# 3dlg-hcvc/minsu3d

Hardware: AMD Instinct MI355X
Metric: scenes/sec (fwd+bwd) PointGroup on ~150k-pt 2cm voxels (higher is better)
Workload: dtype f32; 1 GPU; PointGroup m=16, synthetic ScanNet-shaped scenes (~144k points, ~106k voxels @2cm each), 4 scenes/GPU/step, grouping+ScoreNet branch on, fwd+loss+bwd+Adam; scenes_per_gpu=4, parallelism=dp1, grouping_inputs=GT labels, GT offsets + N(0,4cm) (random-init net groups nothing)

## Files before the change

minsu3d_amd/csrc/spconv.hip:

```cpp
#include <stdlib.h>
#include <atomic>
#include <map>
#include <mutex>
#include <unordered_map>
#include "common.h"
#include "../../include/minsu3d_hip.h"

typedef float f32x4 __attribute__((ext_vector_type(4)));

namespace {

constexpr int MAX_NBT = 8;
constexpr size_t LDS_BUDGET = 150 * 1024;
static hipError_t raise_lds_ceiling(const void *fn)
{
    hipFuncAttributes fa;
    hipError_t e = hipFuncGetAttributes(&fa, fn);
    if (e != hipSuccess) return e;
    return hipFuncSetAttribute(fn, hipFuncAttributeMaxDynamicSharedMemorySize, 160 * 1024 - (int)fa.sharedSizeBytes);
}

int env_int(const char *name, int dflt)
{
    const char *e = getenv(name);
    return e ? atoi(e) : dflt;
}

struct ConvArgs {
    const float *in;
    const float *wf;
    const float *wfs;
    const void *wfb;
    const int *nbr;
    float *out;
    const float *pre_scale;
    const float *pre_shift;
    const float *residual;
    const float *bias;
    const float *bn_x;
    const float *bn_scale;
    const float *bn_shift;
    const float *bn_mean;
    const float *bn_invstd;
    float *bn_partial;
    int out_stats;
    int Vout, K, Cin, Cout;
    int NCH;
    int NBtot;
    int G;
    int GC;
    int RT;
    int ntiles;
    int pre_relu;
    const int *pl_tile_start;
    const int *pl_entries;
    int dyn_picks;
    int k1_path;
    float *ws_slabs;
    unsigned *ws_cnt;
    int ws_ng, ws_kg, ws_R, ws_tpp;
};

__device__ __forceinline__ long stream_slot(long o, int NBtot)
{
    const int lane = (int)(o & 63);
    long r = o >> 6;
    const int nb = (int)(r % NBtot); r /= NBtot;
    const int t = (int)(r & 3); r >>= 2;
    return ((r * NBtot + nb) * 64 + lane) * 4 + t;
}

typedef __bf16 bf16x8 __attribute__((ext_vector_type(8)));

__host__ __device__ constexpr int aux_pieces(int aux_kind) { return aux_kind == 2 ? 3 : aux_kind == 3 ? 2 : aux_kind == 4 ? 1 : 0; }

__host__ __device__ inline bool bf3_dims_ok(int K, int Cin, int Cout)
{
    return K > 1 && Cin % 16 == 0 && Cout % 16 == 0 && Cin >= 48 && Cout >= 48 && Cin <= 256 && Cout <= 256;
}
// ... 417 lines not shown
{
    __syncthreads();
    float *dst = p.bn_partial + ((size_t)blockIdx.y * gridDim.x + blockIdx.x) * 2 * p.Cout;
    for (int t = threadIdx.x; t < 2 * p.Cout; t += blockDim.x) {
        const int which = t >= p.Cout, c = t - which * p.Cout - 16 * nb0;
        float sum = 0.f;
        if (c >= 0 && c < NBT * 16)
            for (int w = 0; w < nslots; w++) sum += s_part[(size_t)w * stat_slot_floats(NBT) + which * NBT * 16 + c];
        dst[t] = sum;
    }
}

template <int NBT>
__device__ __forceinline__ void store_tile(const ConvArgs &p, int row0, int nb0, f32x4 (&acc)[NBT], float *slot)
{
    const int l = lane_id(), q = l >> 4, jl = l & 15;
#pragma unroll
    for (int nb = 0; nb < NBT; nb++) {
        const int j = 16 * (nb0 + nb) + jl;
        const bool j_ok = j < p.Cout;
        float s1 = 0.f, s2 = 0.f;
#pragma unroll
        for (int r = 0; r < 4; r++) {
            const int row = row0 + 4 * q + r;
            if (row < p.Vout && j_ok) {
                float v = acc[nb][r];
                const size_t o = (size_t)row * p.Cout + j;
                if (p.residual) v += p.residual[o];
                if (p.bias) v += p.bias[j];
                if (p.bn_x) {
                    const float x = p.bn_x[o];
                    const float z = fmaf(x, p.bn_scale[j], p.bn_shift[j]);
                    v = (z > 0.f) ? v : 0.f;
                    s1 += v;
                    s2 += v * ((x - p.bn_mean[j]) * p.bn_invstd[j]);
                } else if (p.out_stats) {
                    s1 += v;
                    s2 = fmaf(v, v, s2);
                }
                p.out[o] = v;
            }
        }
        if (p.bn_x || p.out_stats) {
            s1 += __shfl_xor(s1, 16, 64); s1 += __shfl_xor(s1, 32, 64);
            s2 += __shfl_xor(s2, 16, 64); s2 += __shfl_xor(s2, 32, 64);
            if (q == 0) {
                slot[16 * nb + jl] += s1;
                slot[NBT * 16 + 16 * nb + jl] += s2;
            }
        }
    }
}

template <int NBT, bool ALIGNED, bool RES>
__global__ __launch_bounds__(1024) void spconv_fwd_kernel(ConvArgs p)
{
    extern __shared__ float lds[];
    const int l = lane_id(), q = l >> 4;
    const int waves = blockDim.x >> 6;
    const int nb0 = blockIdx.y * NBT;
    float *sW = lds;
    float *s_part = lds + (size_t)p.G * p.NCH * 4 * NBT * 64;
    const int slab4 = NBT * 16;
    auto stage = [&](int k_lo, int cnt) {
        const int rows = cnt * p.NCH * 4;
        for (int e = threadIdx.x; e < rows * slab4; e += blockDim.x) {
            const int r = e / slab4, c4 = e - r * slab4;
            reinterpret_cast<f32x4 *>(sW)[e] =
                reinterpret_cast<const f32x4 *>(p.wf + ((size_t)k_lo * p.NCH * 4 + r) * p.NBtot * 64 + (size_t)nb0 * 64)[c4];
        }
    };

    const bool with_partial = p.bn_x != nullptr || p.out_stats != 0;
    if (with_partial) stats_clear<NBT>(s_part, waves);
    float *slot = s_part + (size_t)wave_id() * stat_slot_floats(NBT);
    const int nblk = gridDim.x;
    const int per_xcd = (nblk + 7) / 8;
    int vb = (blockIdx.x % 8) * per_xcd + blockIdx.x / 8;
    if (nblk % 8 != 0) vb = blockIdx.x;

    if constexpr (RES) {
        stage(0, p.K);
        __syncthreads();
        const int total_waves = nblk * waves;
        const int chunk = (p.ntiles + total_waves - 1) / total_waves;
        const int wglobal = vb * waves + wave_id();
        const int t_begin = wglobal * chunk, t_end = min(p.ntiles, t_begin + chunk);
        for (int tile = t_begin; tile < t_end; tile++) {
            const int row0 = tile * 16;
            const int my_row = row0 + (l & 15);
            f32x4 acc[NBT];
#pragma unroll
            for (int nb = 0; nb < NBT; nb++) acc[nb] = (f32x4){0.f, 0.f, 0.f, 0.f};
            if (p.K == 1 && (p.k1_path & 1)) accumulate_k1<NBT, ALIGNED, false>(p, sW, my_row, q, nb0, acc);
            else accumulate_offsets<NBT, ALIGNED>(p, sW, 0, p.K, 0, my_row, q, nb0, acc);
            ConvArgs pt = p;
            asm volatile("" : "+s"(pt.out), "+s"(pt.residual), "+s"(pt.bias), "+s"(pt.bn_x), "+s"(pt.bn_scale), "+s"(pt.bn_shift),
                         "+s"(pt.bn_mean), "+s"(pt.bn_invstd));
            store_tile<NBT>(pt, row0, nb0, acc, slot);
        }
    } else {
        const int tile = vb * waves + wave_id();
        const int row0 = tile * 16;
        const int my_row = row0 + (l & 15);
        f32x4 acc[NBT];
#pragma unroll
        for (int nb = 0; nb < NBT; nb++) acc[nb] = (f32x4){0.f, 0.f, 0.f, 0.f};
        for (int g0 = 0; g0 < p.K; g0 += p.G) {
            const int gn = min(p.G, p.K - g0);
            __syncthreads();
            stage(g0, gn);
            __syncthreads();
            if (tile < p.ntiles) accumulate_offsets<NBT, ALIGNED>(p, sW, g0, g0 + gn, 0, my_row, q, nb0, acc);
        }
        if (tile < p.ntiles) store_tile<NBT>(p, row0, nb0, acc, slot);
    }
    if (with_partial) stats_flush<NBT>(p, s_part, waves, nb0);
}

constexpr int OGB = 5;

template <int NBT, int OG, int P = 3>
__global__ __launch_bounds__(1024) void spconv_fwd_bf3_kernel(ConvArgs p)
{
    extern __shared__ float lds[];
    const int l = lane_id(), g8 = l >> 4;
    const int waves = blockDim.x >> 6;
    const int nb0 = blockIdx.y * NBT;
    const int NC32 = (p.Cin + 31) >> 5;
    const int GC = p.GC > 0 ? p.GC : NC32;
    uint4 *sW = reinterpret_cast<uint4 *>(lds);
    const int slab = NBT * P * 64;
    float *s_part = lds + (size_t)p.G * GC * slab * 4;
    const uint4 *img = reinterpret_cast<const uint4 *>(p.wfb);
    auto stage = [&](int k_lo, int cnt, int c_lo, int ccnt) {
        uint4 *dst = sW;
        const int chunks = cnt * ccnt * NBT * P;
        for (int ch = wave_id(); ch < chunks; ch += waves) {
            const int r = ch / (NBT * P), within = ch - r * (NBT * P);
            const int kk = r / ccnt, cc = r - kk * ccnt;
            const uint4 *src = img + ((size_t)((k_lo + kk) * NC32 + c_lo + cc) * p.NBtot + nb0) * P * 64 + within * 64 + l;
            __builtin_amdgcn_global_load_lds((const __attribute__((address_space(1))) void *)src,
                                             (__attribute__((address_space(3))) void *)(dst + (size_t)ch * 64), 16, 0, 0);
        }
    };
    const bool with_partial = p.bn_x != nullptr || p.out_stats != 0;
    if (with_partial) stats_clear<NBT>(s_part, waves);
    const int nblk = gridDim.x;
    const int per_xcd = (nblk + 7) / 8;
    int vb = (blockIdx.x % 8) * per_xcd + blockIdx.x / 8;
    if (nblk % 8 != 0) vb = blockIdx.x;
    const bool affine = p.pre_scale != nullptr;
    const float relu_floor = p.pre_relu ? 0.f : -INFINITY;

    auto load_idx = [&](int k0, int k_end, int my_row, int (&idx)[OG]) {
        const bool row_ok = my_row < p.Vout;
        const int safe_row = row_ok ? my_row : 0;
#pragma unroll
        for (int u = 0; u < OG; u++) {
            const int k = min(k0 + u, p.K - 1);
            const int v = p.nbr[(size_t)k * p.Vout + safe_row];
            idx[u] = v | ((row_ok && k0 + u < k_end) ? 0 : -1);
        }
    };
    struct Round { f32x4 lo[OG], hi[OG]; };
    auto gather = [&](int c32, const int (&idx)[OG], Round &r) {
        const int cr = 32 * c32 + 8 * g8;
        const int c0 = cr < p.Cin ? cr : p.Cin - 8;
#pragma unroll
// ... 379 lines not shown
#pragma unroll
        for (int nb = 0; nb < NBT; nb++)
#pragma unroll
            for (int r = 0; r < 4; r++) s_acc[(((size_t)w * RT + t) * NBT + nb) * 256 + r * 64 + l] = acc[t][nb][r];
    __syncthreads();
    for (int t = w; t < RT; t += waves) {
        if (tile0 + t >= p.ntiles) break;
        f32x4 sum[NBT];
#pragma unroll
        for (int nb = 0; nb < NBT; nb++) sum[nb] = (f32x4){0.f, 0.f, 0.f, 0.f};
        for (int ww = 0; ww < waves; ww++)
#pragma unroll
            for (int nb = 0; nb < NBT; nb++)
#pragma unroll
                for (int r = 0; r < 4; r++) sum[nb][r] += s_acc[(((size_t)ww * RT + t) * NBT + nb) * 256 + r * 64 + l];
        store_tile<NBT>(p, (tile0 + t) * 16, nb0, sum, s_part + (size_t)w * stat_slot_floats(NBT));
    }
    if (with_partial) stats_flush<NBT>(p, s_part, waves, nb0);
}

template <int NBT, int RT, int P = 3>
int launch_fwd_small_bf3_rt(const ConvArgs &p, dim3 grid, int threads, size_t lds, hipStream_t stream)
{
    static const hipError_t attr = raise_lds_ceiling((const void *)spconv_fwd_small_bf3_rt_kernel<NBT, RT, P>);
    MS3D_CHECK(attr);
    spconv_fwd_small_bf3_rt_kernel<NBT, RT, P><<<grid, threads, lds, stream>>>(p);
    MS3D_LAUNCH_CHECK();
    return 0;
}

template <int NBT, int P = 3>
int launch_fwd_small_bf3(const ConvArgs &p, dim3 grid, int threads, size_t lds, hipStream_t stream)
{
    spconv_fwd_small_bf3_kernel<NBT, P><<<grid, threads, lds, stream>>>(p);
    MS3D_LAUNCH_CHECK();
    return 0;
}

template <int NBT>
int launch_fwd_small(const ConvArgs &p, dim3 grid, int threads, size_t lds, bool aligned, hipStream_t stream)
{
    if (aligned)
        spconv_fwd_small_kernel<NBT, true><<<grid, threads, lds, stream>>>(p);
    else
        spconv_fwd_small_kernel<NBT, false><<<grid, threads, lds, stream>>>(p);
    MS3D_LAUNCH_CHECK();
    return 0;
}

template <int NBT>
int launch_fwd(const ConvArgs &p, dim3 grid, int threads, size_t lds, bool aligned, hipStream_t stream)
{
    const bool res = p.G >= p.K;
#define MS3D_FWD_LAUNCH(A, R)                                                                                        \
    do {                                                                                                             \
        static const hipError_t attr = raise_lds_ceiling((const void *)spconv_fwd_kernel<NBT, A, R>);                \
        MS3D_CHECK(attr);                                                                                            \
        spconv_fwd_kernel<NBT, A, R><<<grid, threads, lds, stream>>>(p);                                             \
    } while (0)
    if (aligned && res) MS3D_FWD_LAUNCH(true, true);
    else if (aligned) MS3D_FWD_LAUNCH(true, false);
    else if (res) MS3D_FWD_LAUNCH(false, true);
    else MS3D_FWD_LAUNCH(false, false);
#undef MS3D_FWD_LAUNCH
    MS3D_LAUNCH_CHECK();
    return 0;
}


struct WsBlock { int u, g, nb0, k_lo, kcnt, t_begin, t_end; };

template <int NBT>
__device__ __forceinline__ bool ws_block(const ConvArgs &p, WsBlock &b)
{
    const int ny = p.NBtot / NBT, units = p.ws_R * ny;
    const int id = (int)blockIdx.x;
    b.u = (id / (8 * p.ws_ng)) * 8 + (id & 7);
    b.g = (id >> 3) % p.ws_ng;
    if (b.u >= units) return false;
    const int c = b.u % ny, r = b.u / ny;
    b.nb0 = c * NBT;
    b.k_lo = b.g * p.ws_kg;
    b.kcnt = min(p.K, b.k_lo + p.ws_kg) - b.k_lo;
    b.t_begin = r * p.ws_tpp;
    b.t_end = min(p.ntiles, b.t_begin + p.ws_tpp);
    return true;
}

__device__ __forceinline__ f32x4 *ws_slab_ptr(const ConvArgs &p, int g, int tile, int nb)
{
    return reinterpret_cast<f32x4 *>(p.ws_slabs) + (((size_t)g * p.ntiles + tile) * p.NBtot + nb) * 64 + lane_id();
}

template <int NBT>
__device__ __forceinline__ void ws_finish(const ConvArgs &p, const WsBlock &b, float *s_part, int *s_flag)
{
    const int w = wave_id(), waves = blockDim.x >> 6;
    const bool with_partial = p.bn_x != nullptr || p.out_stats != 0;
    if (p.ws_ng > 1) {
        asm volatile("s_waitcnt vmcnt(0)" ::: "memory");
        __syncthreads();
        if (threadIdx.x == 0) {
            __builtin_amdgcn_fence(__ATOMIC_RELEASE, "agent");
            asm volatile("s_waitcnt vmcnt(0)" ::: "memory");
            const unsigned t = __hip_atomic_fetch_add(&p.ws_cnt[b.u], 1u, __ATOMIC_RELAXED, __HIP_MEMORY_SCOPE_AGENT);
            const int last = t == (unsigned)(p.ws_ng - 1);
// ... 1396 lines not shown
#pragma unroll
            for (int b = 0; b < NA; b++)
#pragma unroll
                for (int r = 0; r < 4; r++) dst[b * 256 + r * 64 + l] = acc[b][r];
            if (l == 0) s_pk[w][n_partial] = k;
            n_partial++;
        }
    }
    if (pk0 >= 0) {
#pragma unroll
        for (int b = 0; b < NA; b++)
#pragma unroll
            for (int r = 0; r < 4; r++) s_tile[b * 256 + r * 64 + l] = part0[b][r];
        if (l == 0) s_pk[w][0] = pk0;
    }
    __syncthreads();
    for (int k = w; k < p.K; k += nw) {
        const bool empty = s_cum[k + 1] == s_cum[k];
        f32x4 acc[NA];
#pragma unroll
        for (int b = 0; b < NA; b++) acc[b] = (f32x4){0.f, 0.f, 0.f, 0.f};
        bool any = false;
        for (int ww = 0; ww < nw; ww++)
            for (int jj = 0; jj < 2; jj++)
                if (s_pk[ww][jj] == k) {
                    any = true;
                    const float *src = lds + (size_t)ww * WAVE_KB * 256 + (size_t)jj * NA * 256;
#pragma unroll
                    for (int b = 0; b < NA; b++)
#pragma unroll
                        for (int r = 0; r < 4; r++) acc[b][r] += src[b * 256 + r * 64 + l];
                }
        if (any || empty) store_slab(k, acc);
    }
}

template <int NBT, int NCH, int TB = WGRAD_TB>
int launch_wgrad_offsetlist(const WgradArgs &p, int nblk_rows, hipStream_t stream)
{
    constexpr int wave_kb = TB * (NCH + NBT) > 2 * NCH * NBT ? TB * (NCH + NBT) : 2 * NCH * NBT;
    const size_t per_wave = (size_t)wave_kb * 256 * sizeof(float);
    static const int max_w = env_int("MS3D_WGRAD_LIST_WAVES", 16);
    int nw = (int)(LDS_BUDGET / per_wave);
    if (nw > 16) nw = 16;
    if (nw > max_w && max_w >= 1) nw = max_w;
    dim3 grid(nblk_rows, ms3d_divup(p.NBtot, NBT), ms3d_divup(ms3d_divup(p.Cin, 16), NCH));
    const size_t lds = (size_t)nw * per_wave;
    static const hipError_t attr = raise_lds_ceiling((const void *)spconv_wgrad_offsetlist_kernel<NBT, NCH, TB>);
    MS3D_CHECK(attr);
    spconv_wgrad_offsetlist_kernel<NBT, NCH, TB><<<grid, nw * 64, lds, stream>>>(p);
    MS3D_LAUNCH_CHECK();
    return 0;
}

__global__ __launch_bounds__(1024) void bn_finalize_stats_kernel(const float *__restrict__ partial, int nparts, int C, long V,
                                                                float eps, float momentum, const float *__restrict__ gamma,
                                                                const float *__restrict__ beta, float *running_mean,
                                                                float *running_var, float *__restrict__ mean_out,
                                                                float *__restrict__ invstd_out, float *__restrict__ scale_out,
                                                                float *__restrict__ shift_out)
{
    __shared__ double s_1[16][17], s_2[16][17];
    const int cl = threadIdx.x & 15, lp = threadIdx.x >> 4;
    const int c = blockIdx.x * 16 + cl;
    double a1 = 0.0, a2 = 0.0;
    if (c < C) {
        int p = lp;
        for (; p + 192 < nparts; p += 256) {
            float v1[4], v2[4];
#pragma unroll
            for (int u = 0; u < 4; u++) {
                v1[u] = partial[((size_t)(p + 64 * u) * 2 + 0) * C + c];
                v2[u] = partial[((size_t)(p + 64 * u) * 2 + 1) * C + c];
            }
#pragma unroll
            for (int u = 0; u < 4; u++) {
                a1 += (double)v1[u];
                a2 += (double)v2[u];
            }
        }
        for (; p < nparts; p += 64) {
            a1 += (double)partial[((size_t)p * 2 + 0) * C + c];
            a2 += (double)partial[((size_t)p * 2 + 1) * C + c];
        }
    }
    a1 += __shfl_xor(a1, 16, 64); a2 += __shfl_xor(a2, 16, 64);
    a1 += __shfl_xor(a1, 32, 64); a2 += __shfl_xor(a2, 32, 64);
    if ((threadIdx.x & 63) < 16) {
        s_1[threadIdx.x >> 6][cl] = a1;
        s_2[threadIdx.x >> 6][cl] = a2;
    }
    __syncthreads();
    if (threadIdx.x >= 16 || c >= C) return;
    double s1 = 0.0, s2 = 0.0;
#pragma unroll
    for (int i = 0; i < 16; i++) {
        s1 += s_1[i][cl];
        s2 += s_2[i][cl];
    }
    const double mean = s1 / (double)V;
    double var = s2 / (double)V - mean * mean;
    if (var < 0.0) var = 0.0;
    const float invstd = (float)(1.0 / sqrt(var + (double)eps));
    const float g = gamma ? gamma[c] : 1.f, b = beta ? beta[c] : 0.f;
    mean_out[c] = (float)mean;
    invstd_out[c] = invstd;
// ... 777 lines not shown
int ms3d_spconv_pairlist_rows_dense(int Vout, int K, int Cin, int Cout)
{
    const int plain = ms3d_spconv_pairlist_rows(Vout, K, Cin, Cout);
    static const int narrow = env_int("MS3D_PL_NARROW", 1);
    if (plain != MS3D_PL_ROWS || !narrow || K != 27 || Cin != 32 || Cout != 32) return plain;
    const FwdGeom g = fwd_geometry(Vout, K, Cin, Cout, false, PL_ROWS_NARROW);
    return (g.ok && g.pairlist && g.pl_rows == PL_ROWS_NARROW) ? PL_ROWS_NARROW : plain;
}

int ms3d_spconv_partial_blocks(int Vout, int K, int Cin, int Cout, int with_pairlist)
{
    const FwdGeom g = fwd_geometry(Vout, K, Cin, Cout, true, with_pairlist == 1 ? MS3D_PL_ROWS : with_pairlist);
    return g.nblk * g.ny;
}

static int spconv_forward_impl(const float *in, const float *wf, const int *nbr, int Vout, int K, int Cin, int Cout,
                               float *out, const float *pre_scale, const float *pre_shift, int pre_relu,
                               const float *residual, const float *bn_x, const float *bn_scale, const float *bn_shift,
                               const float *bn_mean, const float *bn_invstd, float *bn_partial, int out_stats,
                               const float *bias, const int *pl_tile_start, const int *pl_entries, const float *wf_aux,
                               int aux_kind, ms3d_stream_t stream_);

int ms3d_spconv_forward(const float *in, const float *wf, const int *nbr, int Vout, int K, int Cin, int Cout,
                        float *out, const float *pre_scale, const float *pre_shift, int pre_relu,
                        const float *residual, const float *bn_x, const float *bn_scale, const float *bn_shift,
                        const float *bn_mean, const float *bn_invstd, float *bn_partial, int out_stats,
                        const float *bias, const int *pl_tile_start, const int *pl_entries, const float *wf_stream,
                        ms3d_stream_t stream_)
{
    return spconv_forward_impl(in, wf, nbr, Vout, K, Cin, Cout, out, pre_scale, pre_shift, pre_relu, residual, bn_x, bn_scale,
                               bn_shift, bn_mean, bn_invstd, bn_partial, out_stats, bias, pl_tile_start, pl_entries,
                               wf_stream, wf_stream ? 1 : 0, stream_);
}

static int spconv_forward_impl(const float *in, const float *wf, const int *nbr, int Vout, int K, int Cin, int Cout,
                               float *out, const float *pre_scale, const float *pre_shift, int pre_relu,
                               const float *residual, const float *bn_x, const float *bn_scale, const float *bn_shift,
                               const float *bn_mean, const float *bn_invstd, float *bn_partial, int out_stats,
                               const float *bias, const int *pl_tile_start, const int *pl_entries, const float *wf_stream,
                               int aux_kind, ms3d_stream_t stream_)
{
    hipStream_t stream = (hipStream_t)stream_;
    if (Vout <= 0) return 0;
    ConvArgs p;
    p.bias = bias;
    p.wfs = nullptr;
    p.wfb = nullptr;
    const int pieces = aux_pieces(aux_kind);
    if (aux_kind != 1 && !pieces) wf_stream = nullptr;
    p.pl_tile_start = pl_tile_start; p.pl_entries = pl_entries;
    p.out_stats = (out_stats && bn_partial && !bn_x) ? 1 : 0;
    static const int dyn_picks = [] { const char *e = getenv("MS3D_PL_DYNAMIC"); return e ? atoi(e) : 0; }();
    p.dyn_picks = dyn_picks;
    static const int k1_path = [] { const char *e = getenv("MS3D_K1_PATH"); return e ? atoi(e) : 3; }();
    p.k1_path = k1_path;
    p.in = in; p.wf = wf; p.nbr = nbr; p.out = out; p.pre_scale = pre_scale; p.pre_shift = pre_shift;
    p.residual = residual; p.bn_x = bn_x; p.bn_scale = bn_scale; p.bn_shift = bn_shift; p.bn_mean = bn_mean;
    p.bn_invstd = bn_invstd; p.bn_partial = bn_partial; p.Vout = Vout; p.K = K; p.Cin = Cin; p.Cout = Cout;
    p.NCH = ms3d_divup(Cin, 16); p.NBtot = ms3d_divup(Cout, 16); p.ntiles = ms3d_divup(Vout, 16); p.pre_relu = pre_relu;
    FwdPlan pl;
    const int rc = fwd_plan(Vout, K, Cin, Cout, (pl_tile_start && pl_entries) ? ms3d_kmap_pairlist_rows_of(pl_tile_start) : 0,
                            wf_stream ? aux_kind : 0, bn_x != nullptr || p.out_stats, pl);
    if (rc != 0) return rc;
    const FwdGeom &g = pl.g;
    p.G = pl.G;
    p.GC = pl.GC;
    p.RT = g.small ? g.rt : 1;
    dim3 grid(pl.grid_x, g.ny);
    const bool aligned = (Cin % 16 == 0);
    p.ws_slabs = nullptr; p.ws_cnt = nullptr; p.ws_ng = p.ws_kg = p.ws_R = p.ws_tpp = 0;
#define MS3D_BF_NBT(LAUNCH, P_, ...)                                                                                   \
    switch (g.nbt) {                                                                                                   \
        case 2: return LAUNCH<2, ##__VA_ARGS__, P_>(p, grid, g.threads, pl.lds, stream);                              \
        case 3: return LAUNCH<3, ##__VA_ARGS__, P_>(p, grid, g.threads, pl.lds, stream);                              \
        case 4: return LAUNCH<4, ##__VA_ARGS__, P_>(p, grid, g.threads, pl.lds, stream);                              \
        case 5: return LAUNCH<5, ##__VA_ARGS__, P_>(p, grid, g.threads, pl.lds, stream);                              \
        case 6: return LAUNCH<6, ##__VA_ARGS__, P_>(p, grid, g.threads, pl.lds, stream);                              \
        case 7: return LAUNCH<7, ##__VA_ARGS__, P_>(p, grid, g.threads, pl.lds, stream);                              \
        case 8: return LAUNCH<8, ##__VA_ARGS__, P_>(p, grid, g.threads, pl.lds, stream);                              \
    }
#define MS3D_BF_P(LAUNCH, ...)                                                                                         \
    if (pieces == 3) { MS3D_BF_NBT(LAUNCH, 3, ##__VA_ARGS__) }                                                         \
    else if (pieces == 2) { MS3D_BF_NBT(LAUNCH, 2, ##__VA_ARGS__) }                                                    \
    else { MS3D_BF_NBT(LAUNCH, 1, ##__VA_ARGS__) }
#define MS3D_F32_NBT(LAUNCH)                                                                                           \
    switch (g.nbt) {                                                                                                   \
        case 1: return LAUNCH<1>(p, grid, g.threads, pl.lds, aligned, stream);                                        \
        case 2: return LAUNCH<2>(p, grid, g.threads, pl.lds, aligned, stream);                                        \
        case 3: return LAUNCH<3>(p, grid, g.threads, pl.lds, aligned, stream);                                        \
        case 4: return LAUNCH<4>(p, grid, g.threads, pl.lds, aligned, stream);                                        \
        case 5: return LAUNCH<5>(p, grid, g.threads, pl.lds, aligned, stream);                                        \
        case 6: return LAUNCH<6>(p, grid, g.threads, pl.lds, aligned, stream);                                        \
        case 7: return LAUNCH<7>(p, grid, g.threads, pl.lds, aligned, stream);                                        \
        case 8: return LAUNCH<8>(p, grid, g.threads, pl.lds, aligned, stream);                                        \
    }
    switch (pl.family) {
        case FWD_WS: {
            WsSpace *sp = ws_space(stream, g.ws_ng > 1 ? (size_t)g.ws_ng * p.ntiles * p.NBtot * 256 : 0, g.ws_R * g.ny);
            if (!sp) return (int)hipErrorOutOfMemory;
            p.ws_slabs = sp->slabs; p.ws_cnt = sp->cnt;
            p.ws_ng = g.ws_ng; p.ws_kg = g.ws_kg; p.ws_R = g.ws_R; p.ws_tpp = g.ws_tpp;
            switch (g.nbt) {
                case 1: return launch_fwd_ws<1>(p, pl.grid_x, g.threads, pl.lds, stream);
                case 2: return launch_fwd_ws<2>(p, pl.grid_x, g.threads, pl.lds, stream);
                case 3: return launch_fwd_ws<3>(p, pl.grid_x, g.threads, pl.lds, stream);
                case 4: return launch_fwd_ws<4>(p, pl.grid_x, g.threads, pl.lds, stream);
            }
// ... 263 lines not shown
    int rc = wgrad_plan(Vout, K, Cin, Cout, ol_kt_start && ol_entries, submanifold, precision, plan);
    if (rc) return rc;
    const bool use_list = plan.route == WGRAD_LIST, wide2 = plan.wide2;
    p.ol_kt_start = ol_kt_start; p.ol_entries = ol_entries;
    p.rows_per_block = plan.rows_per_block;
    int nblk = plan.nblk;
    const int nb = p.NBtot;
    if (use_list) {
        const int nbs = nb <= 4 ? nb : ms3d_divup(nb, ms3d_divup(nb, 4));
        const bool two = ms3d_divup(Cin, 16) % 2 == 0 && nbs <= 2;
        rc = nbs == 1 ? (two ? launch_wgrad_offsetlist<1, 2>(p, nblk, stream) : launch_wgrad_offsetlist<1, 1>(p, nblk, stream))
           : nbs == 2 ? (two ? launch_wgrad_offsetlist<2, 2>(p, nblk, stream) : launch_wgrad_offsetlist<2, 1>(p, nblk, stream))
           : nbs == 3 ? launch_wgrad_offsetlist<3, 1>(p, nblk, stream)
                      : (wide2 ? launch_wgrad_offsetlist<4, 2, 1>(p, nblk, stream) : launch_wgrad_offsetlist<4, 1>(p, nblk, stream));
        if (rc) return rc;
        if (defer_nblk) { *defer_nblk = nblk; return 0; }
        launch_wgrad_reduce(partial_ws, nblk, n, dW, stream);
        MS3D_LAUNCH_CHECK();
        return 0;
    }
    if (plan.route == WGRAD_BF16) {
        const int P = 3 - precision;
        float *base = partial_ws + ms3d_spconv_wgrad_slab_floats(Vout, K, Cin, Cout);
        bf16x8 *img = reinterpret_cast<bf16x8 *>((reinterpret_cast<uintptr_t>(base) + 15) & ~(uintptr_t)15);
        const long ntile = ms3d_divup(Vout, 32);
        bf16x8 *xs = img + (size_t)ntile * nb * P * 64;
        const long t1 = ntile * nb * 64, t2 = (long)Vout * (Cin / 8);
        const int nb1 = (int)((t1 + 255) / 256), nb2 = (int)((t2 + 255) / 256);
        if (P == 3)
            wgrad_bf3_operands_kernel<3><<<nb1 + nb2, 256, 0, stream>>>(dout, in, Vout, Cin, Cout, nb, ntile, nb1, pre_scale,
                                                                       pre_shift, pre_relu, img, xs);
        else if (P == 2)
            wgrad_bf3_operands_kernel<2><<<nb1 + nb2, 256, 0, stream>>>(dout, in, Vout, Cin, Cout, nb, ntile, nb1, pre_scale,
                                                                       pre_shift, pre_relu, img, xs);
        else
            wgrad_bf3_operands_kernel<1><<<nb1 + nb2, 256, 0, stream>>>(dout, in, Vout, Cin, Cout, nb, ntile, nb1, pre_scale,
                                                                       pre_shift, pre_relu, img, xs);
        MS3D_LAUNCH_CHECK();
        WgradBf3Args q;
        q.xs = xs; q.dout_img = img; q.nbr = nbr; q.partial = partial_ws; q.Vout = Vout; q.K = K; q.Cin = Cin; q.Cout = Cout;
        q.NBtot = nb;
        q.rows_per_block = plan.rows_per_block;
#define MS3D_WG_BF(P_)                                                                                                 \
    (nb == 3 ? launch_wgrad_bf3<14, 3, 1, P_>(q, nblk, stream) : nb == 4 ? launch_wgrad_bf3<9, 4, 1, P_>(q, nblk, stream)   \
     : nb <= 6 ? launch_wgrad_bf3<9, 3, 2, P_>(q, nblk, stream) : launch_wgrad_bf3<9, 4, 2, P_>(q, nblk, stream))
        rc = P == 3 ? MS3D_WG_BF(3) : P == 2 ? MS3D_WG_BF(2) : MS3D_WG_BF(1);
#undef MS3D_WG_BF
        if (rc) return rc;
        if (defer_nblk) { *defer_nblk = nblk; return 0; }
        launch_wgrad_reduce(partial_ws, nblk, n, dW, stream);
        MS3D_LAUNCH_CHECK();
        return 0;
    }
    if (nb == 1) rc = (K >= 27) ? launch_wgrad<9, 1>(p, nblk, stream, dl) : launch_wgrad<8, 1>(p, nblk, stream, dl);
    else if (nb == 2) rc = (K >= 27) ? launch_wgrad<9, 2>(p, nblk, stream, dl) : launch_wgrad<8, 2>(p, nblk, stream, dl);
    else if (nb == 3) rc = (K >= 27) ? launch_wgrad<9, 3>(p, nblk, stream, dl) : launch_wgrad<8, 3>(p, nblk, stream, dl);
    else if (nb == 4) rc = launch_wgrad<4, 4>(p, nblk, stream, dl);
    else if (nb == 5) rc = launch_wgrad<4, 5>(p, nblk, stream, dl);
    else if (nb == 6) rc = launch_wgrad<4, 6>(p, nblk, stream, dl);
    else if (nb == 7) rc = launch_wgrad<4, 7>(p, nblk, stream, dl);
    else if (nb == 8) rc = launch_wgrad<3, 8>(p, nblk, stream, dl);
    else if (nb <= 10) rc = launch_wgrad<2, 10>(p, nblk, stream, dl);
    else if (nb <= 12) rc = launch_wgrad<2, 12>(p, nblk, stream, dl);
    else rc = launch_wgrad<2, 14>(p, nblk, stream, dl);
    if (rc) return rc;
    if (defer_nblk) { *defer_nblk = nblk; return 0; }
    launch_wgrad_reduce(partial_ws, nblk, n, dW, stream);
    MS3D_LAUNCH_CHECK();
    return 0;
}

size_t ms3d_spconv_wgrad_launch_bytes(void) { return 128; }

int ms3d_spconv_wgrad_multi(const void *descs, int n_desc, int total_blocks, int variant, ms3d_stream_t stream_)
{
    hipStream_t stream = (hipStream_t)stream_;
    if (n_desc <= 0 || total_blocks <= 0) return 0;
    switch (variant) {
#define MS3D_WM(KG, NBT) case KG * 100 + NBT: return launch_wgrad_multi<KG, NBT>(descs, n_desc, total_blocks, stream);
        MS3D_WM(9, 1) MS3D_WM(8, 1) MS3D_WM(9, 2) MS3D_WM(8, 2) MS3D_WM(9, 3) MS3D_WM(8, 3) MS3D_WM(4, 4) MS3D_WM(4, 5)
        MS3D_WM(4, 6) MS3D_WM(4, 7) MS3D_WM(3, 8) MS3D_WM(2, 10) MS3D_WM(2, 12) MS3D_WM(2, 14)
#undef MS3D_WM
    }
    return MS3D_E_UNSUPPORTED;
}

int ms3d_wgrad_reduce_blocks(long n, const float *slabs, const float *dW, int *wide)
{
    const bool w = n >= 32768 && (n & 3) == 0 && ((uintptr_t)slabs & 15) == 0 && ((uintptr_t)dW & 15) == 0;
    if (wide) *wide = w ? 1 : 0;
    return w ? ms3d_divup(n / 4, 64) : ms3d_divup(n, 16);
}

int ms3d_wgrad_reduce_multi(const void *descs, int n_desc, int total_blocks, ms3d_stream_t stream)
{
    if (n_desc <= 0 || total_blocks <= 0) return 0;
    wgrad_reduce_multi_kernel<<<total_blocks, 256, 0, (hipStream_t)stream>>>(static_cast<const WgradReduceDesc *>(descs),
                                                                           n_desc);
    MS3D_LAUNCH_CHECK();
    return 0;
}

int ms3d_bn_stats(const float *x, long V, int C, float eps, float momentum, const float *gamma, const float *beta,
                  float *running_mean, float *running_var, float *mean, float *invstd, float *scale, float *shift,
                  float *partial_ws, int partial_rows, ms3d_stream_t stream_)
{
    hipStream_t stream = (hipStream_t)stream_;
    if (V <= 0) return MS3D_E_UNSUPPORTED;
    int nblk = (int)((V + 255) / 256);
    if (nblk > partial_rows) nblk = partial_rows;
    if (nblk < 1) nblk = 1;
    const int rows_per_block = (int)((V + nblk - 1) / nblk);
    const int rc = launch_bn_partial_stats(x, V, C, partial_ws, nblk, rows_per_block, stream);
    if (rc) return rc;
    bn_finalize_stats_kernel<<<ms3d_divup(C, 16), 1024, 0, stream>>>(partial_ws, nblk, C, V, eps, momentum, gamma, beta,
                                                                  running_mean, running_var, mean, invstd, scale, shift);
    MS3D_LAUNCH_CHECK();
    return 0;
}

int ms3d_column_sum(const float *x, long V, int C, float *partial_ws, int partial_rows, float *out2c, ms3d_stream_t stream_)
{
    hipStream_t stream = (hipStream_t)stream_;
    if (V <= 0) {
        MS3D_CHECK(hipMemsetAsync(out2c, 0, sizeof(float) * 2 * C, stream));
        return 0;
    }
    int nblk = (int)((V + 1023) / 1024);
    if (nblk > partial_rows) nblk = partial_rows;
    if (nblk < 1) nblk = 1;
    const int rows_per_block = (int)((V + nblk - 1) / nblk);
    const int rc = launch_bn_partial_stats(x, V, C, partial_ws, nblk, rows_per_block, stream);
    if (rc) return rc;
    return ms3d_reduce_partials(partial_ws, nblk, 2 * C, out2c, stream_);
}
// ... 293 lines not shown
```

Baseline: 204.2 scenes/sec.

## Add dedicated software-pipelined kernels for 1x1 sparse conv forward and weight grad

Adds specialised kernels for K=1 (pointwise) sparse convolutions. In forward, each wave handles a contiguous chunk of tiles with weights staged in LDS once, and prefetches the next tile's neighbour index and input rows while the current tile runs MFMA. In weight-grad, a 4-wave kernel double-buffers gathered input and dout rows and reduces across waves in LDS. Both are turned on by default through a new k1_path default of 15. The cost is more code and template instances, and the forward uses a different grid mapping that could hurt occupancy.

```diff
diff --git a/minsu3d_amd/csrc/spconv.hip b/minsu3d_amd/csrc/spconv.hip
--- a/minsu3d_amd/csrc/spconv.hip
+++ b/minsu3d_amd/csrc/spconv.hip
@@ -25,6 +25,7 @@
     const char *e = getenv(name);
     return e ? atoi(e) : dflt;
 }
+constexpr int MS3D_K1_PATH_DEFAULT = 15;
 
 struct ConvArgs {
     const float *in;
@@ -548,6 +549,183 @@
     }
 }
 
+template <int NBT, bool ALIGNED>
+__device__ __forceinline__ void k1_tile_loop(const ConvArgs &p, const float *__restrict__ sW, int t_begin, int t_end, int nb0,
+                                             float *slot)
+{
+    constexpr int CB = 4;
+    const int l = lane_id(), q = l >> 4, i = l & 15;
+    if (t_begin >= t_end) return;
+    int opaque0 = 0;
+    asm volatile("" : "+s"(opaque0));
+    const bool wide = (p.Cout & 3) == 0 &&
+                      ((reinterpret_cast<uintptr_t>(p.out) | reinterpret_cast<uintptr_t>(p.residual) |
+                        reinterpret_cast<uintptr_t>(p.bn_x) | reinterpret_cast<uintptr_t>(p.bias) |
+                        reinterpret_cast<uintptr_t>(p.bn_scale) | reinterpret_cast<uintptr_t>(p.bn_shift) |
+                        reinterpret_cast<uintptr_t>(p.bn_mean) | reinterpret_cast<uintptr_t>(p.bn_invstd)) & 15) == 0;
+    auto entry = [&](int tile) -> int {
+        const int row = tile * 16 + i;
+        return p.nbr[min(row, p.Vout - 1)] | (row < p.Vout ? 0 : -1);
+    };
+    auto fetch = [&](int idx, int ch0, f32x4 (&a)[CB]) {
+        const float *row = p.in + (size_t)max(idx, 0) * p.Cin + 4 * q;
+#pragma unroll
+        for (int u = 0; u < CB; u++) {
+            const int ch = min(ch0 + u, p.NCH - 1);
+            if (ALIGNED) {
+                a[u] = *reinterpret_cast<const f32x4 *>(row + 16 * ch);
+            } else {
+#pragma unroll
+                for (int t = 0; t < 4; t++) a[u][t] = (16 * ch + 4 * q + t < p.Cin) ? row[16 * ch + t] : 0.f;
+            }
+        }
+    };
+    auto multiply = [&](int ch0, f32x4 (&a)[CB], int keep, f32x4 (&acc)[NBT]) {
+#pragma unroll
+        for (int u = 0; u < CB; u++) {
+            if (ch0 + u >= p.NCH) break;
+            const int ch = ch0 + u, c0 = 16 * ch + 4 * q;
+            if (p.pre_scale) {
+                f32x4 sc, sh;
+                if (ALIGNED) {
+                    sc = *reinterpret_cast<const f32x4 *>(p.pre_scale + c0);
+                    sh = *reinterpret_cast<const f32x4 *>(p.pre_shift + c0);
+                } else {
+#pragma unroll
+                    for (int t = 0; t < 4; t++) {
+                        sc[t] = (c0 + t < p.Cin) ? p.pre_scale[c0 + t] : 0.f;
+                        sh[t] = (c0 + t < p.Cin) ? p.pre_shift[c0 + t] : 0.f;
+                    }
+                }
+#pragma unroll
+                for (int t = 0; t < 4; t++) {
+                    const float v = fmaf(a[u][t], sc[t], sh[t]);
+                    a[u][t] = p.pre_relu ? fmaxf(v, 0.f) : v;
+                }
+            }
+#pragma unroll
+            for (int t = 0; t < 4; t++) a[u][t] = __int_as_float(__float_as_int(a[u][t]) & keep);
+            const float *w = sW + (size_t)(ch * 4) * NBT * 64 + l;
+#pragma unroll
+            for (int t = 0; t < 4; t++)
+#pragma unroll
+                for (int nb = 0; nb < NBT; nb++)
+                    acc[nb] = __builtin_amdgcn_mfma_f32_16x16x4f32(w[(t * NBT + nb) * 64], a[u][t], acc[nb], 0, 0, 0);
+        }
+    };
+    f32x4 st1[NBT], st2[NBT];
+#pragma unroll
+    for (int nb = 0; nb < NBT; nb++) st1[nb] = st2[nb] = (f32x4){0.f, 0.f, 0.f, 0.f};
+
+    int idx_n = entry(t_begin);
+    f32x4 a_n[CB];
+    fetch(idx_n, 0, a_n);
+    int idx_nn = entry(t_begin + 1 + opaque0);
+    for (int tile = t_begin; tile < t_end; tile++) {
+        const int idx = idx_n, keep = ~(idx >> 31);
+        f32x4 a[CB];
+#pragma unroll
+        for (int u = 0; u < CB; u++) a[u] = a_n[u];
+        idx_n = idx_nn;
+        fetch(idx_n, 0, a_n);
+        idx_nn = entry(tile + 2 + opaque0);
+        const int row = tile * 16 + i;
+        const bool row_ok = row < p.Vout;
+        const size_t orow = (size_t)min(row, p.Vout - 1) * p.Cout;
+        f32x4 acc[NBT];
+#pragma unroll
+        for (int nb = 0; nb < NBT; nb++) acc[nb] = (f32x4){0.f, 0.f, 0.f, 0.f};
+        if (__ballot(idx >= 0) != 0ull) {
+            multiply(0, a, keep, acc);
+            for (int ch0 = CB; ch0 < p.NCH; ch0 += CB) {
+                f32x4 b[CB];
+                fetch(idx, ch0, b);
+                multiply(ch0, b, keep, acc);
+            }
+        }
+        f32x4 res[NBT], bx[NBT];
+        if (wide) {
+#pragma unroll
+            for (int nb = 0; nb < NBT; nb++) {
+                const int j0 = 16 * (nb0 + nb) + 4 * q, js = j0 < p.Cout ? j0 : 0;
+                if (p.residual) res[nb] = *reinterpret_cast<const f32x4 *>(p.residual + orow + js);
+                if (p.bn_x) bx[nb] = *reinterpret_cast<const f32x4 *>(p.bn_x + orow + js);
+            }
+        }
+#pragma unroll
+        for (int nb = 0; nb < NBT; nb++) {
+            const int j0 = 16 * (nb0 + nb) + 4 * q;
+            if (wide) {
+                if (row_ok && j0 < p.Cout) {
+                    f32x4 v = acc[nb];
+                    if (p.residual) v += res[nb];
+                    if (p.bias) v += *reinterpret_cast<const f32x4 *>(p.bias + j0);
+                    if (p.bn_x) {
+                        const f32x4 sc = *reinterpret_cast<const f32x4 *>(p.bn_scale + j0);
+                        const f32x4 sh = *reinterpret_cast<const f32x4 *>(p.bn_shift + j0);
+                        const f32x4 mu = *reinterpret_cast<const f32x4 *>(p.bn_mean + j0);
+                        const f32x4 is = *reinterpret_cast<const f32x4 *>(p.bn_invstd + j0);
+#pragma unroll
+                        for (int r = 0; r < 4; r++) {
+                            const float x = bx[nb][r];
+                            const float z = fmaf(x, sc[r], sh[r]);
+                            v[r] = (z > 0.f) ? v[r] : 0.f;
+                            st1[nb][r] += v[r];
+                            st2[nb][r] += v[r] * ((x - mu[r]) * is[r]);
+                        }
+                    } else if (p.out_stats) {
+#pragma unroll
+                        for (int r = 0; r < 4; r++) {
+                            st1[nb][r] += v[r];
+                            st2[nb][r] = fmaf(v[r], v[r], st2[nb][r]);
+                        }
+                    }
+                    *reinterpret_cast<f32x4 *>(p.out + orow + j0) = v;
+                }
+            } else {
+#pragma unroll
+                for (int r = 0; r < 4; r++) {
+                    const int j = j0 + r;
+                    if (row_ok && j < p.Cout) {
+                        float v = acc[nb][r];
+                        const size_t o = orow + j;
+                        if (p.residual) v += p.residual[o];
+                        if (p.bias) v += p.bias[j];
+                        if (p.bn_x) {
+                            const float x = p.bn_x[o];
+                            const float z = fmaf(x, p.bn_scale[j], p.bn_shift[j]);
+                            v = (z > 0.f) ? v : 0.f;
+                            st1[nb][r] += v;
+                            st2[nb][r] += v * ((x - p.bn_mean[j]) * p.bn_invstd[j]);
+                        } else if (p.out_stats) {
+                            st1[nb][r] += v;
+                            st2[nb][r] = fmaf(v, v, st2[nb][r]);
+                        }
+                        p.out[o] = v;
+                    }
+                }
+            }
+        }
+    }
+    if (p.bn_x || p.out_stats) {
+#pragma unroll
+        for (int nb = 0; nb < NBT; nb++)
+#pragma unroll
+            for (int r = 0; r < 4; r++) {
+                float s1 = st1[nb][r], s2 = st2[nb][r];
+#pragma unroll
+                for (int m = 1; m < 16; m <<= 1) {
+                    s1 += __shfl_xor(s1, m, 64);
+                    s2 += __shfl_xor(s2, m, 64);
+                }
+                if (i == 0) {
+                    slot[16 * nb + 4 * q + r] += s1;
+                    slot[NBT * 16 + 16 * nb + 4 * q + r] += s2;
+                }
+            }
+    }
+}
+
 template <int NBT, bool ALIGNED, bool RES>
 __global__ __launch_bounds__(1024) void spconv_fwd_kernel(ConvArgs p)
 {
@@ -611,6 +789,37 @@
         }
         if (tile < p.ntiles) store_tile<NBT>(p, row0, nb0, acc, slot);
     }
+    if (with_partial) stats_flush<NBT>(p, s_part, waves, nb0);
+}
+
+constexpr int K1_LOOP_MAX_THREADS = 512;
+constexpr bool k1_loop_serves(int nbt) { return nbt == 1 || nbt == 2 || nbt == 4; }
+template <int NBT, bool ALIGNED>
+__global__ __launch_bounds__(K1_LOOP_MAX_THREADS, NBT <= 2 ? 4 : 2) void spconv_fwd_k1_kernel(ConvArgs p)
+{
+    extern __shared__ float lds[];
+    const int waves = blockDim.x >> 6;
+    const int nb0 = blockIdx.y * NBT;
+    float *sW = lds;
+    float *s_part = lds + (size_t)p.NCH * 4 * NBT * 64;
+    const int rows = p.NCH * 4, slab4 = NBT * 16;
+    for (int e = threadIdx.x; e < rows * slab4; e += blockDim.x) {
+        const int r = e / slab4, c4 = e - r * slab4;
+        reinterpret_cast<f32x4 *>(sW)[e] = reinterpret_cast<const f32x4 *>(p.wf + (size_t)r * p.NBtot * 64 + (size_t)nb0 * 64)[c4];
+    }
+    const bool with_partial = p.bn_x != nullptr || p.out_stats != 0;
+    if (with_partial) stats_clear<NBT>(s_part, waves);
+    float *slot = s_part + (size_t)wave_id() * stat_slot_floats(NBT);
+    const int nblk = gridDim.x;
+    const int per_xcd = (nblk + 7) / 8;
+    int vb = (blockIdx.x % 8) * per_xcd + blockIdx.x / 8;
+    if (nblk % 8 != 0) vb = blockIdx.x;
+    __syncthreads();
+    const int total_waves = nblk * waves;
+    const int chunk = (p.ntiles + total_waves - 1) / total_waves;
+    const int wglobal = vb * waves + wave_id();
+    const int t_begin = wglobal * chunk, t_end = min(p.ntiles, t_begin + chunk);
+    k1_tile_loop<NBT, ALIGNED>(p, sW, t_begin, t_end, nb0, slot);
     if (with_partial) stats_flush<NBT>(p, s_part, waves, nb0);
 }
 
@@ -1096,6 +1305,14 @@
 int launch_fwd(const ConvArgs &p, dim3 grid, int threads, size_t lds, bool aligned, hipStream_t stream)
 {
     const bool res = p.G >= p.K;
+    if constexpr (k1_loop_serves(NBT)) {
+        if (res && p.K == 1 && (p.k1_path & 5) == 5 && threads <= K1_LOOP_MAX_THREADS && lds <= 64 * 1024) {
+            if (aligned) spconv_fwd_k1_kernel<NBT, true><<<grid, threads, lds, stream>>>(p);
+            else spconv_fwd_k1_kernel<NBT, false><<<grid, threads, lds, stream>>>(p);
+            MS3D_LAUNCH_CHECK();
+            return 0;
+        }
+    }
 #define MS3D_FWD_LAUNCH(A, R)                                                                                        \
     do {                                                                                                             \
         static const hipError_t attr = raise_lds_ceiling((const void *)spconv_fwd_kernel<NBT, A, R>);                \
@@ -2598,6 +2815,223 @@
     MS3D_LAUNCH_CHECK();
     return 0;
 }
+
+constexpr int WGRAD_K1_WAVES = 4;
+constexpr int wgrad_k1_tb(int nbt, int nch) { return nch + nbt >= 6 ? 1 : 2; }
+constexpr int wgrad_k1_wave_kb(int nbt, int nch)
+{
+    return wgrad_k1_tb(nbt, nch) * (nch + nbt) > nch * nbt ? wgrad_k1_tb(nbt, nch) * (nch + nbt) : nch * nbt;
+}
+constexpr int wgrad_k1_variant(int nbt, int nch) { return 10000 + nch * 100 + nbt; }
+
+template <int NBT, int NCH>
+__device__ __forceinline__ void wgrad_k1_body(const WgradArgs &p, const int bx, const int bz, float *lds)
+{
+    constexpr int TB = wgrad_k1_tb(NBT, NCH), NT = NCH + NBT, NA = NCH * NBT, WAVE_KB = wgrad_k1_wave_kb(NBT, NCH);
+    constexpr int nw = WGRAD_K1_WAVES;
+    const int l = lane_id(), q = l >> 4, cl = l & 15, w = wave_id();
+    float *s_tile = lds + (size_t)w * WAVE_KB * 256;
+    const int qs = q ^ ((cl >> 1) & 3);
+    const int cbase = bz * NCH * 16;
+    const bool vec = ((p.Cin | p.Cout) & 3) == 0 &&
+                     ((reinterpret_cast<uintptr_t>(p.in) | reinterpret_cast<uintptr_t>(p.dout)) & 15) == 0;
+    f32x4 sc[NCH], sh[NCH];
+#pragma unroll
+    for (int ch = 0; ch < NCH; ch++)
+#pragma unroll
+        for (int i = 0; i < 4; i++) {
+            const int c = cbase + 16 * ch + 4 * q + i;
+            const bool ok = p.pre_scale && c < p.Cin;
+            sc[ch][i] = ok ? p.pre_scale[c] : 1.f;
+            sh[ch][i] = ok ? p.pre_shift[c] : 0.f;
+        }
+    const int r_begin = bx * p.rows_per_block;
+    const int r_end = min(p.Vout, r_begin + p.rows_per_block);
+    const int nbatch = (r_end - r_begin + 15) >> 4;
+    int opaque0 = 0;
+    asm volatile("" : "+s"(opaque0));
+    f32x4 acc[NA];
+#pragma unroll
+    for (int b = 0; b < NA; b++) acc[b] = (f32x4){0.f, 0.f, 0.f, 0.f};
+
+    int e[TB], erow[TB];
+    int gk[TB], grow[TB];
+    f32x4 ga[TB][NCH], gb[TB][NBT];
+    auto load_entries = [&](int bt) {
+#pragma unroll
+        for (int t = 0; t < TB; t++) {
+            erow[t] = min(r_begin + 16 * (bt + t) + cl, r_end - 1);
+            e[t] = p.nbr[erow[t]];
+        }
+    };
+    auto gather = [&]() {
+#pragma unroll
+        for (int t = 0; t < TB; t++) {
+            gk[t] = e[t];
+            grow[t] = erow[t];
+            const float *xi = p.in + (size_t)max(e[t], 0) * p.Cin;
+            const float *dy = p.dout + (size_t)erow[t] * p.Cout;
+            if (vec) {
+#pragma unroll
+                for (int ch = 0; ch < NCH; ch++) {
+                    const int c0 = cbase + 16 * ch + 4 * q;
+                    ga[t][ch] = *reinterpret_cast<const f32x4 *>(xi + (c0 < p.Cin ? c0 : 0));
+                }
+#pragma unroll
+                for (int nb = 0; nb < NBT; nb++) {
+                    const int j0 = 16 * nb + 4 * q;
+                    gb[t][nb] = *reinterpret_cast<const f32x4 *>(dy + (j0 < p.Cout ? j0 : 0));
+                }
+            } else {
+#pragma unroll
+                for (int ch = 0; ch < NCH; ch++)
+#pragma unroll
+                    for (int i = 0; i < 4; i++) ga[t][ch][i] = xi[min(cbase + 16 * ch + 4 * q + i, p.Cin - 1)];
+#pragma unroll
+                for (int nb = 0; nb < NBT; nb++)
+#pragma unroll
+                    for (int i = 0; i < 4; i++) gb[t][nb][i] = dy[min(16 * nb + 4 * q + i, p.Cout - 1)];
+            }
+        }
+    };
+    const int step = nw * TB, bt0 = w * TB;
+    if (bt0 < nbatch) {
+        load_entries(bt0);
+        gather();
+        load_entries(bt0 + step + opaque0);
+    }
+    for (int bt = bt0; bt < nbatch; bt += step) {
+        f32x4 ca[TB][NCH], cb[TB][NBT];
+        int ck[TB], crow[TB];
+#pragma unroll
+        for (int t = 0; t < TB; t++) {
+            ck[t] = gk[t];
+            crow[t] = grow[t];
+#pragma unroll
+            for (int ch = 0; ch < NCH; ch++) ca[t][ch] = ga[t][ch];
+#pragma unroll
+            for (int nb = 0; nb < NBT; nb++) cb[t][nb] = gb[t][nb];
+        }
+        gather();
+        load_entries(bt + 2 * step + opaque0);
+#pragma unroll
+        for (int t = 0; t < TB; t++) {
+            const bool row_ok = r_begin + 16 * (bt + t) + cl == crow[t];
+            const bool in_ok = row_ok && ck[t] >= 0;
+            float *ta = s_tile + (size_t)t * NT * 256;
+#pragma unroll
+            for (int ch = 0; ch < NCH; ch++) {
+#pragma unroll
+                for (int i = 0; i < 4; i++) {
+                    float v = ca[t][ch][i];
+                    if (p.pre_scale) {
+                        v = fmaf(v, sc[ch][i], sh[ch][i]);
+                        if (p.pre_relu) v = fmaxf(v, 0.f);
+                    }
+                    ca[t][ch][i] = (in_ok && cbase + 16 * ch + 4 * q + i < p.Cin) ? v : 0.f;
+                }
+                *reinterpret_cast<f32x4 *>(ta + ch * 256 + cl * 16 + 4 * qs) = ca[t][ch];
+            }
+#pragma unroll
+            for (int nb = 0; nb < NBT; nb++) {
+#pragma unroll
+                for (int i = 0; i < 4; i++) cb[t][nb][i] = (row_ok && 16 * nb + 4 * q + i < p.Cout) ? cb[t][nb][i] : 0.f;
+                *reinterpret_cast<f32x4 *>(ta + (NCH + nb) * 256 + cl * 16 + 4 * qs) = cb[t][nb];
+            }
+        }
+#pragma unroll
+        for (int t = 0; t < TB; t++) {
+            const float *ta = s_tile + (size_t)t * NT * 256;
+#pragma unroll
+            for (int st = 0; st < 4; st++) {
+                const int o = (4 * st + q) * 16 + (cl ^ (((2 * st + (q >> 1)) & 3) << 2));
+                float bv[NBT];
+#pragma unroll
+                for (int nb = 0; nb < NBT; nb++) bv[nb] = ta[(NCH + nb) * 256 + o];
+#pragma unroll
+                for (int ch = 0; ch < NCH; ch++) {
+                    const float av = ta[ch * 256 + o];
+#pragma unroll
+                    for (int nb = 0; nb < NBT; nb++)
+                        acc[ch * NBT + nb] = __builtin_amdgcn_mfma_f32_16x16x4f32(av, bv[nb], acc[ch * NBT + nb], 0, 0, 0);
+                }
+            }
+        }
+    }
+#pragma unroll
+    for (int b = 0; b < NA; b++)
+#pragma unroll
+        for (int r = 0; r < 4; r++) s_tile[b * 256 + r * 64 + l] = acc[b][r];
+    __syncthreads();
+    float *dst = p.partial + (size_t)bx * p.Cin * p.Cout;
+    for (int o = threadIdx.x; o < NA * 256; o += nw * 64) {
+        float v = 0.f;
+#pragma unroll
+        for (int ww = 0; ww < nw; ww++) v += lds[(size_t)ww * WAVE_KB * 256 + o];
+        const int b = o >> 8, r = (o >> 6) & 3, ln = o & 63;
+        const int ci = cbase + 16 * (b / NBT) + 4 * (ln >> 4) + r, j = 16 * (b % NBT) + (ln & 15);
+        if (ci < p.Cin && j < p.Cout) dst[(size_t)ci * p.Cout + j] = v;
+    }
+}
+
+template <int NBT, int NCH>
+__global__ __launch_bounds__(64 * WGRAD_K1_WAVES) void spconv_wgrad_k1_kernel(WgradArgs p, const unsigned char *__restrict__ descs,
+                                                                              int n_desc)
+{
+    extern __shared__ float lds[];
+    int bx = blockIdx.x, bz = blockIdx.z;
+    if (descs) {
+        int lo = 0, hi = n_desc - 1;
+        const int blk = blockIdx.x;
+        while (lo < hi) {
+            const int mid = (lo + hi + 1) >> 1;
+            if (reinterpret_cast<const WgradLaunch *>(descs + 128 * (size_t)mid)->block_begin <= blk) lo = mid; else hi = mid - 1;
+        }
+        const WgradLaunch *d = reinterpret_cast<const WgradLaunch *>(descs + 128 * (size_t)lo);
+        const int local = blk - d->block_begin;
+        bx = local % d->gx;
+        bz = local / (d->gx * d->gy);
+        p = d->p;
+    }
+    wgrad_k1_body<NBT, NCH>(p, bx, bz, lds);
+}
+
+template <int NBT, int NCH>
+int launch_wgrad_k1(const WgradArgs &p, int nblk_rows, hipStream_t stream, WgradLaunch *defer = nullptr)
+{
+    dim3 grid(nblk_rows, 1, ms3d_divup(ms3d_divup(p.Cin, 16), NCH));
+    if (defer) {
+        defer->block_begin = 0;
+        defer->gx = grid.x; defer->gy = grid.y; defer->gz = grid.z;
+        defer->variant = wgrad_k1_variant(NBT, NCH);
+        defer->nblk = nblk_rows;
+        defer->p = p;
+        return 0;
+    }
+    const size_t lds = (size_t)WGRAD_K1_WAVES * wgrad_k1_wave_kb(NBT, NCH) * 1024;
+    spconv_wgrad_k1_kernel<NBT, NCH><<<grid, 64 * WGRAD_K1_WAVES, lds, stream>>>(p, nullptr, 0);
+    MS3D_LAUNCH_CHECK();
+    return 0;
+}
+
+template <int NBT, int NCH>
+int launch_wgrad_k1_multi(const void *descs, int n_desc, int total_blocks, hipStream_t stream)
+{
+    const size_t lds = (size_t)WGRAD_K1_WAVES * wgrad_k1_wave_kb(NBT, NCH) * 1024;
+    WgradArgs none = {};
+    spconv_wgrad_k1_kernel<NBT, NCH><<<total_blocks, 64 * WGRAD_K1_WAVES, lds, stream>>>(none, static_cast<const unsigned char *>(descs),
+                                                                                       n_desc);
+    MS3D_LAUNCH_CHECK();
+    return 0;
+}
+
+static int wgrad_k1_nch(int Cin, int nb)
+{
+    if (nb > 8) return 0;
+    const int cap = nb <= 2 ? 4 : nb <= 4 ? 2 : 1, nch = ms3d_divup(Cin, 16);
+    return nch >= 4 ? cap : nch >= 2 ? (cap < 2 ? cap : 2) : 1;
+}
+#define MS3D_WK1_ALL(X) X(1, 1) X(1, 2) X(1, 4) X(2, 1) X(2, 2) X(2, 4) X(3, 1) X(3, 2) X(4, 1) X(4, 2) X(5, 1) X(6, 1) X(7, 1) X(8, 1)
 
 __global__ __launch_bounds__(1024) void bn_finalize_stats_kernel(const float *__restrict__ partial, int nparts, int C, long V,
                                                                 float eps, float momentum, const float *__restrict__ gamma,
@@ -3481,7 +3915,7 @@
     p.out_stats = (out_stats && bn_partial && !bn_x) ? 1 : 0;
     static const int dyn_picks = [] { const char *e = getenv("MS3D_PL_DYNAMIC"); return e ? atoi(e) : 0; }();
     p.dyn_picks = dyn_picks;
-    static const int k1_path = [] { const char *e = getenv("MS3D_K1_PATH"); return e ? atoi(e) : 3; }();
+    static const int k1_path = env_int("MS3D_K1_PATH", MS3D_K1_PATH_DEFAULT);
     p.k1_path = k1_path;
     p.in = in; p.wf = wf; p.nbr = nbr; p.out = out; p.pre_scale = pre_scale; p.pre_shift = pre_shift;
     p.residual = residual; p.bn_x = bn_x; p.bn_scale = bn_scale; p.bn_shift = bn_shift; p.bn_mean = bn_mean;
@@ -3851,6 +4285,19 @@
         MS3D_LAUNCH_CHECK();
         return 0;
     }
+    static const int k1_path = env_int("MS3D_K1_PATH", MS3D_K1_PATH_DEFAULT);
+    const int k1_nch = (K == 1 && (k1_path & 8)) ? wgrad_k1_nch(Cin, nb) : 0;
+    if (k1_nch) {
+        rc = MS3D_E_UNSUPPORTED;
+#define MS3D_WK1(NBT_, NCH_) if (nb == NBT_ && k1_nch == NCH_) rc = launch_wgrad_k1<NBT_, NCH_>(p, nblk, stream, dl);
+        MS3D_WK1_ALL(MS3D_WK1)
+#undef MS3D_WK1
+        if (rc) return rc;
+        if (defer_nblk) { *defer_nblk = nblk; return 0; }
+        launch_wgrad_reduce(partial_ws, nblk, n, dW, stream);
+        MS3D_LAUNCH_CHECK();
+        return 0;
+    }
     if (nb == 1) rc = (K >= 27) ? launch_wgrad<9, 1>(p, nblk, stream, dl) : launch_wgrad<8, 1>(p, nblk, stream, dl);
     else if (nb == 2) rc = (K >= 27) ? launch_wgrad<9, 2>(p, nblk, stream, dl) : launch_wgrad<8, 2>(p, nblk, stream, dl);
     else if (nb == 3) rc = (K >= 27) ? launch_wgrad<9, 3>(p, nblk, stream, dl) : launch_wgrad<8, 3>(p, nblk, stream, dl);
@@ -3880,6 +4327,9 @@
         MS3D_WM(9, 1) MS3D_WM(8, 1) MS3D_WM(9, 2) MS3D_WM(8, 2) MS3D_WM(9, 3) MS3D_WM(8, 3) MS3D_WM(4, 4) MS3D_WM(4, 5)
         MS3D_WM(4, 6) MS3D_WM(4, 7) MS3D_WM(3, 8) MS3D_WM(2, 10) MS3D_WM(2, 12) MS3D_WM(2, 14)
 #undef MS3D_WM
+#define MS3D_WK1(NBT_, NCH_) case wgrad_k1_variant(NBT_, NCH_): return launch_wgrad_k1_multi<NBT_, NCH_>(descs, n_desc, total_blocks, stream);
+        MS3D_WK1_ALL(MS3D_WK1)
+#undef MS3D_WK1
     }
     return MS3D_E_UNSUPPORTED;
 }
```

Result: slower. 193.7 scenes/sec (-5.1%).
